# tiantianxuabc/ORB_SLAM2_Refactored

Hardware: AMD Instinct MI355X
Metric: frames/sec ORB extract+match (1280×720, 8 lvl, 1000 feat) + LocalBA iters/sec (higher is better)
Workload: dtype u8; 1 GPU; C2: 1280x720 mono, 8 levels, 2000 features, extract + brute-force Hamming top-2/ratio match of every frame vs its predecessor; width=1280, height=720, nlevels=8, nfeatures=2000, parallelism=8192-frame job sharded over 1 GPU(s), 8192 frames per GPU

## Files before the change

orb_slam2_refactored_amd/csrc/orbx.hip:

```cpp
#include <algorithm>
#include <cfloat>
#include <cmath>
#include <cstring>
#include <mutex>
#include <type_traits>
#include <vector>

#include <hip/hip_ext.h>

#include "common.h"
#include "qt_sort.h"
#include "sincos_f.h"
#include "stereo.h"

namespace orbamd {

constexpr int MAX_LEVELS = 16;
constexpr int MAX_ZONE = 64;
constexpr int MAX_ROOTS = 32;
constexpr int PATCH = 43;
constexpr int HBLUR_W = 37;
constexpr int HBS = 40;
static_assert(HBLUR_W + 3 <= HBS, "the blur's fourth-column tiles store up to column 39");

// ... 2693 lines not shown
        asm volatile("s_waitcnt vmcnt(0) lgkmcnt(0)\n\ts_nop 7\n\ts_nop 7" ::: "memory");
#endif
        const i4v cinit = {128 * 256, 128 * 256, 128 * 256, 128 * 256};
        i4v acc[3][3];
#pragma unroll
        for (int nt = 0; nt < 3; nt++)
#pragma unroll
            for (int mt = 0; mt < 3; mt++)
#if DESC_HBT
                acc[nt][mt] = __builtin_amdgcn_mfma_i32_16x16x64_i8(bfr[nt], afr[mt], cinit, 0, 0, 0);
#else
                acc[nt][mt] = __builtin_amdgcn_mfma_i32_16x16x64_i8(afr[mt], bfr[nt], cinit, 0, 0, 0);
#endif
#if defined(DESC_DIAG_NOPS) && DESC_DIAG_NOPS == 2
        asm volatile("s_waitcnt vmcnt(0) lgkmcnt(0)\n\ts_nop 7\n\ts_nop 7\n\ts_nop 7" ::: "memory");
#endif
#ifdef DESC_KEEPALIVE_DIAG
        asm volatile("" ::"v"(bfr[0]), "v"(bfr[1]), "v"(bfr[2]));
        asm volatile("" ::"v"(afr[0]), "v"(afr[1]), "v"(afr[2]));
#endif
        auto put = [&](int nt, int mt) {
            uint2 pk;
            pk.x = __builtin_amdgcn_perm((uint32_t)acc[nt][mt].y, (uint32_t)acc[nt][mt].x, 0x05040100u);
            pk.y = __builtin_amdgcn_perm((uint32_t)acc[nt][mt].w, (uint32_t)acc[nt][mt].z, 0x05040100u);
#if DESC_HBT
            *reinterpret_cast<uint2*>(&Hb[(16 * mt + n) * HCS + 16 * nt + 4 * lg]) = pk;
#else
            *reinterpret_cast<uint2*>(&Hb[(16 * nt + n) * HBS + 16 * mt + 4 * lg]) = pk;
#endif
        };
#pragma unroll
        for (int nt = 0; nt < 3; nt++) {
            put(nt, 0);
            put(nt, 1);
        }
#if DESC_HBT
        if (n < 8) {
#else
        if (lg < 2) {
#endif
#pragma unroll
            for (int nt = 0; nt < 3; nt++) put(nt, 2);
        }
    }

#if DESC_PAT_EARLY
    float4 pat[4];
#pragma unroll
    for (int r = 0; r < 4; r++) pat[r] = __builtin_bit_cast(float4, tab16(DT_PAT + 1024 * r));
#endif
#if DESC_ANGLE_MFMA && !DESC_ANGLE_FIRST
    {
        i4v au[3], av[3];
#pragma unroll
        for (int nt = 0; nt < 3; nt++) {
            au[nt] = tab16(DT_AN + 1024 * (2 * nt));
            av[nt] = tab16(DT_AN + 1024 * (2 * nt + 1));
        }
        angle_products(au, av);
    }
#endif
    const float angle = fast_atan2_dev((float)m01, (float)m10);
    DESC_STAMP(2);
    __syncthreads();

    const float factorPI = (float)(M_PI / 180.f);
    const float ang = angle * factorPI;
    float a, b;
    DESC_STAMP(3);
#ifdef DESC_SINCOS_COST_DIAG
    a = __cosf(ang);
    b = __sinf(ang);
#else
    if (TRIG) sincosf_glibc(ang, &b, &a);
    else sincos_f2d_k(ang, &b, &a, c_sincos_k);
#endif
    DESC_STAMP(4);
    auto sample = [&](float x, float y) -> int {
        const float dy = rintf(x * b + y * a), dx = rintf(x * a - y * b);
#if DESC_HBT
        const int q = (int)fmaf(dx, (float)HCS, dy + (float)(18 * HCS + 18));
        const uint32_t* cw = reinterpret_cast<const uint32_t*>(Hb) + (q >> 1);
        const uint32_t d0 = cw[0], d1 = cw[1], d2 = cw[2], d3 = cw[3];
        const uint32_t sh = (uint32_t)(q & 1) * 2u;
        const us2 p01 = u2us(__builtin_amdgcn_alignbyte(d1, d0, sh));
        const us2 p23 = u2us(__builtin_amdgcn_alignbyte(d2, d1, sh));
        const us2 p45 = u2us(__builtin_amdgcn_alignbyte(d3, d2, sh));
        const us2 p6x = u2us(__builtin_amdgcn_alignbyte(d3, d3, sh));
        const us2 k01 = {18, 34}, k23 = {48, 56}, k45 = {48, 34}, k6x = {18, 0};
        unsigned acc = __builtin_amdgcn_udot2(p6x, k6x, 1u << 15, false);
        acc = __builtin_amdgcn_udot2(p01, k01, acc, false);
        acc = __builtin_amdgcn_udot2(p23, k23, acc, false);
        acc = __builtin_amdgcn_udot2(p45, k45, acc, false);
        return (int)(acc >> 16);
#else
        const int ob = (int)fmaf(dy, (float)(2 * HBS), fmaf(dx, 2.f, (float)(2 * (18 * HBS + 18))));
        const uint16_t* col = reinterpret_cast<const uint16_t*>(reinterpret_cast<const uint8_t*>(Hb) + ob);
        const us2 p01 = {col[0], col[HBS]}, p23 = {col[2 * HBS], col[3 * HBS]}, p45 = {col[4 * HBS], col[5 * HBS]};
        const us2 k01 = {18, 34}, k23 = {48, 56}, k45 = {48, 34};
        unsigned acc = __builtin_amdgcn_udot2(p01, k01, 18u * col[6 * HBS] + (1u << 15), false);
        acc = __builtin_amdgcn_udot2(p23, k23, acc, false);
        acc = __builtin_amdgcn_udot2(p45, k45, acc, false);
        return (int)(acc >> 16);
#endif
    };
    unsigned long long words[4];
#pragma unroll
    for (int r = 0; r < 4; r++) {
#if DESC_PAT_EARLY
        const float4 q = pat[r];
#else
        const float4 q = __builtin_bit_cast(float4, tab16(DT_PAT + 1024 * r));
#endif
        words[r] = __ballot(sample(q.x, q.y) < sample(q.z, q.w));
    }
    DESC_STAMP(5);
    uint32_t dv = 0, kv = 0;
#pragma unroll
    for (int r = 0; r < 4; r++) {
        dv = writelane_u32((uint32_t)words[r], 2 * r, dv);
        dv = writelane_u32((uint32_t)(words[r] >> 32), 2 * r + 1, dv);
    }
    const float ks = l > 0 ? L.scale : 1.f;
    kv = writelane_u32(__float_as_uint((float)kx * ks), 0, kv);
    kv = writelane_u32(__float_as_uint((float)ky * ks), 1, kv);
    kv = writelane_u32(__float_as_uint(L.size), 2, kv);
    kv = writelane_u32(__float_as_uint(angle), 3, kv);
    kv = writelane_u32(__float_as_uint((float)score), 4, kv);
    kv = writelane_u32((uint32_t)l, 5, kv);
    kv = writelane_u32(0xffffffffu, 6, kv);
    if (lane < 8) reinterpret_cast<uint32_t*>(desc + o * 32)[lane] = dv;
    if (lane < 7) reinterpret_cast<uint32_t*>(kps + o)[lane] = kv;
    DESC_STAMP(6);
}

#ifndef DESC_SLOT_TAB
#define DESC_SLOT_TAB 1
#endif
constexpr int LVP = 32;

__global__ __launch_bounds__(256) void describe_prefix_kernel(const int* __restrict__ sel_cnt, int nl, int F,
                                                              int* __restrict__ lvl_pre, int32_t* __restrict__ counts,
                                                              int* __restrict__ stat) {
    const int f = blockIdx.x * blockDim.x + threadIdx.x;
    if (f >= F) return;
    int acc = 0;
    int* pre = lvl_pre + (long long)f * LVP;
    for (int q = 0; q < nl; q++) {
        pre[q] = acc;
        acc += sel_cnt[f * nl + q];
    }
    pre[nl] = acc;
    counts[f] = acc;
    atomicMax(stat, acc);
}

struct DescGrid {
    int C;
    unsigned m;
    int s1, s2;
};
template <int TRIG>
__device__ __forceinline__ void describe_dense_slot(const Geom& g, int f, int s, const uint8_t* __restrict__ in,
                                                    long long in_fstride, int in_step, const uint8_t* __restrict__ pyr,
                                                    const uint32_t* __restrict__ sel, orbx_keypoint* __restrict__ kps,
                                                    uint8_t* __restrict__ desc, int cap, const int* __restrict__ lvl_pre,
                                                    uint16_t* Hb, int lb) {
    const int lane = threadIdx.x, nl = g.nlevels;
    const int pq = lane <= nl ? lvl_pre[(long long)f * LVP + lane] : 0x7fffffff;
    const int T = __builtin_amdgcn_readlane(pq, nl);
    if (s >= T || s >= cap) return;
    const int l = popc64(__ballot(lane >= 1 && lane <= nl && pq <= s));
    const int pre_l = __builtin_amdgcn_readlane(pq, l);
    const uint32_t k = sel[(long long)f * g.out_frame + g.lv[l].out_base + (s - pre_l)];
    describe_keypoint<TRIG>(g, l, f, k, (long long)f * cap + s, in, in_fstride, in_step, pyr, kps, desc, Hb, lb);
}

template <int TRIG>
__global__ __launch_bounds__(64) void describe_overflow_kernel(Geom g, const uint8_t* __restrict__ in,
                                                               long long in_fstride, int in_step,
                                                               const uint8_t* __restrict__ pyr,
                                                               const uint32_t* __restrict__ sel,
                                                               orbx_keypoint* __restrict__ kps,
                                                               uint8_t* __restrict__ desc, int cap,
                                                               const int* __restrict__ lvl_pre, int F, int C) {
    __shared__ __attribute__((aligned(16))) uint16_t Hb[HB_ELEMS];
    for (int f = blockIdx.x; f < F; f += gridDim.x) {
        const int T = min(lvl_pre[(long long)f * LVP + g.nlevels], cap);
        for (int s = C; s < T; s++) {
            describe_dense_slot<TRIG>(g, f, s, in, in_fstride, in_step, pyr, sel, kps, desc, cap, lvl_pre, Hb,
                                      (int)blockIdx.x);
            __syncthreads();
        }
    }
}

template <int TRIG>
__global__ __launch_bounds__(64) void describe_kernel(Geom g, const uint8_t* __restrict__ in, long long in_fstride,
                                                      int in_step, const uint8_t* __restrict__ pyr,
                                                      const uint32_t* __restrict__ sel,
                                                      const int* __restrict__ sel_cnt, orbx_keypoint* __restrict__ kps,
                                                      uint8_t* __restrict__ desc, int32_t* __restrict__ counts,
                                                      int cap, const uint32_t* __restrict__ slot_tab,
                                                      const int* __restrict__ lvl_pre, DescGrid dg) {
    __shared__ __attribute__((aligned(16))) uint16_t Hb[HB_ELEMS];
    static_assert(47 * RS + 64 <= HB_ELEMS * 2, "R (and the blur's reads of rows 43..47) must fit in Hb");
    const int lane = threadIdx.x;
    const int lb = xcd_swizzle(blockIdx.x + gridDim.x * blockIdx.y, gridDim.x * gridDim.y);
    DESC_STAMP(7);
    if (dg.C > 0) {
        const unsigned t = __umulhi((unsigned)lb, dg.m);
        const int fd = (int)((t + (((unsigned)lb - t) >> dg.s1)) >> dg.s2);
        (void)sel_cnt; (void)counts; (void)slot_tab;
        describe_dense_slot<TRIG>(g, fd, lb - fd * dg.C, in, in_fstride, in_step, pyr, sel, kps, desc, cap, lvl_pre, Hb,
                                  lb);
        return;
    }
    const int f = divmod_of(g, lb);
    const int s = lb - f * g.out_frame;
#if DESC_SLOT_TAB
    (void)sel_cnt;
    (void)counts;
    (void)lane;
    const uint32_t e = slot_tab[s];
    const uint32_t k = sel[(long long)f * g.out_frame + s];
    asm volatile("" ::"s"(e), "s"(k), "s"(cap), "s"(in), "s"(in_fstride), "s"(in_step), "s"(pyr), "s"(g.pyr_frame_bytes));
    const int l = (int)(e & 255u), i = (int)(e >> 8);
    const int2 pr = *reinterpret_cast<const int2*>(lvl_pre + (long long)f * LVP + l);
    {
        const LevelDev& L = g.lv[l];
        asm volatile("" ::"s"(pr.x), "s"(pr.y), "s"(L.w), "s"(L.h), "s"(L.stride), "s"(L.off));
    }
    if (i >= pr.y - pr.x) return;
    const int oidx = pr.x + i;
    if (oidx >= cap) return;
#else
    (void)slot_tab;
    (void)lvl_pre;
    const int nl = g.nlevels;
    const uint32_t k = sel[(long long)f * g.out_frame + s];
    const int* cf = sel_cnt + f * nl;
    int cnt16[MAX_LEVELS];
#pragma unroll
    for (int q = 0; q < MAX_LEVELS; q++) cnt16[q] = cf[q];
    int l = MAX_LEVELS;
    {
        const unsigned s1 = (unsigned)(s + 1) * 0x00010001u;
#pragma unroll
        for (int d = 0; d < MAX_LEVELS / 2; d++) l -= __popc(((g.lv_start[d] | 0x80008000u) - s1) & 0x80008000u);
    }
    int total = 0, lbase = 0, cnt_l = 0;
#pragma unroll
    for (int q = 0; q < MAX_LEVELS; q++) {
        const int cq = q < nl ? cnt16[q] : 0;
        total += cq;
        lbase += q < l ? cq : 0;
        cnt_l = q == l ? cq : cnt_l;
    }
    if (s == 0 && lane == 0) counts[f] = total;
    const int i = s - g.lv[l].out_base;
    if (i >= cnt_l) return;
    const int oidx = lbase + i;
    if (oidx >= cap) return;
#endif
    describe_keypoint<TRIG>(g, l, f, k, (long long)f * cap + oidx, in, in_fstride, in_step, pyr, kps, desc, Hb, lb);
}

__global__ __launch_bounds__(256) void qt_sort_test_kernel(QtItem* items, int n, int* scratch) {
    __shared__ int s_cnt[2];
    qt_sort_block<false>(items, n, scratch, scratch + n, scratch + 2 * n, scratch + 3 * n,
                  reinterpret_cast<QtItem*>(scratch + 4 * n), scratch + 6 * n, n / 3 + 2, s_cnt);
}

}

using namespace orbamd;

struct orbx_extractor {
    orbx_params p;
    int device = 0;
    hipStream_t stream = nullptr;
    std::vector<float> scale, inv_scale, sigma2, inv_sigma2;
    std::vector<int> quota;
    std::mutex mu;

    int g_rows = -1, g_cols = -1;
    Geom geom;
    std::vector<CellDev> cells;
    int NC = 0, PTC = 0;
    size_t qt_lds = 0;
    int qt_ptc0 = 0;
    size_t qt_lds0 = 0;
    int qt_wave = 0, qt_wave_wg = 2, qtw_l0 = 0, qtw_nc = 0, qtw_ptc = 0;
    size_t qtw_lds = 0;
    FastLds fl;
    size_t fast_lds = 0;
    int fast_cpw = 16;
    int fast_spec = 8;
    int fast_pair = 0;
    bool fast_pair_on = false;
    int fast_spec_first = 1;
    int nsub = 1;
    int debug_nc = 0;
    int debug_qt_block = 0;
    uint32_t fault_host = 0;
    int pyr_mfma = 0;
    std::vector<char> pyr_mfma_ok;
    DevBuf d_pyrmt, d_pyrkb;
    int pyr_pair = 2;
    int trig_float = 0;
    int resize_simd = 0;
    std::vector<std::pair<hipStream_t, hipEvent_t>> sub;
    hipEvent_t fork_ev = nullptr;
    bool lvl_overlap = false;
    hipStream_t lvl_side = nullptr;
    hipEvent_t lvl_fork = nullptr, lvl_join = nullptr;
    DevBuf d_cells, d_xtab, d_ytab;
    DevBuf d_strips;
    DevBuf d_slottab;
    DevBuf d_lvlpre;
    std::vector<int> strip_beg;

    int ws_frames = 0;
    DevBuf d_pyr, d_slots, d_cellcnt, d_P, d_T, d_sel, d_selcnt, d_fault;
    DevBuf d_img, d_kps, d_desc, d_counts;
    DevBuf d_stereo_sad;
    int prof = 0;
    std::vector<std::pair<hipEvent_t, hipEvent_t>> prof_ev[4];
    std::vector<hipEvent_t> ev_pool;
    const uint8_t* last_in = nullptr;
    long long last_fstride = 0;
    size_t last_step = 0;
    int last_frames = 0;
    int desc_dense = 0;
    int desc_force_c = 0;
    int desc_c = 0;
    DevBuf d_dstat;
    int32_t* h_dstat = nullptr;
    hipEvent_t dstat_ev = nullptr;
    bool dstat_pending = false;
    bool last_single = false;
    int last_kcap = 0;
    DevBuf d_stereo_out;
    std::vector<uint8_t> h_stage;
};

static int resize_tail_x(int w, int V) {
    if (V <= 0) return w;
    if (V == 1) return 0;
    int x = 0;
    for (; x <= w - V; x += V) {}
    for (; x < w - V / 2; x += V / 2) {}
    return x;
}

static int cv_round_d(double v) { return (int)std::lrint(v); }
static int cv_round_f(float v) { return (int)std::lrintf(v); }

static void compute_tables(orbx_extractor* h) {
    const orbx_params& p = h->p;
    const int L = p.nlevels;
    h->scale.resize(L); h->inv_scale.resize(L); h->sigma2.resize(L); h->inv_sigma2.resize(L);
    h->quota.resize(L);
    float s = 1.f;
    for (int l = 0; l < L; l++) {
        h->scale[l] = s;
        h->inv_scale[l] = 1.f / s;
        h->sigma2[l] = s * s;
        h->inv_sigma2[l] = 1.f / (s * s);
        s *= p.scaleFactor;
    }
    const double factor = 1 / p.scaleFactor;
    double nf = p.nfeatures * (1 - factor) / (1 - std::pow(factor, L));
    int sum = 0;
    for (int l = 0; l < L - 1; l++) {
        h->quota[l] = cv_round_d(nf);
        sum += h->quota[l];
        nf *= factor;
    }
    h->quota[L - 1] = std::max(p.nfeatures - sum, 0);
}

static int setup_geometry(orbx_extractor* h, int rows, int cols) {
    if (h->g_rows == rows && h->g_cols == cols) return ORB_OK;
    const int Lc = h->p.nlevels;
    Geom g;
    std::memset(&g, 0, sizeof(g));
    g.nlevels = Lc;
    for (int l = Lc; l < MAX_LEVELS; l++) g.lv[l].out_base = INT_MAX;
    std::vector<int2> xtab, ytab;
    std::vector<PyrMfmaLane> mt;
    std::vector<int> mkb;
    std::vector<CellDev> cells;
    long long pyr_off = 0, slot = 0, cand = 0;
    int out = 0, NC = 64;
    int prev_w = cols, prev_h = rows;
    for (int l = 0; l < Lc; l++) {
        LevelDev& L = g.lv[l];
        if (l == 0) {
            L.w = cols; L.h = rows; L.stride = cols; L.off = -1; L.tail_x = cols; L.mt_off = -1;
        } else {
            L.h = cv_round_f(h->inv_scale[l] * rows);
            L.w = cv_round_f(h->inv_scale[l] * cols);
            if (L.w <= 0 || L.h <= 0) {
                set_error("pyramid level collapses to zero size");
                return ORB_EINVAL;
            }
            L.stride = (int)align_up(L.w, 16);
            L.off = pyr_off;
            pyr_off += (long long)align_up((size_t)L.stride * L.h, 256);
            const int sw = prev_w, sh = prev_h, dw = L.w, dh = L.h;
            const double scale_x = 1. / ((double)dw / sw), scale_y = 1. / ((double)dh / sh);
            L.xtab_off = (int)xtab.size();
            L.ytab_off = (int)ytab.size();
            L.ssx = (double)sw / L.w;
            L.ssy = (double)sh / L.h;
            L.tail_x = resize_tail_x(L.w, h->resize_simd);
            int xmax = dw;
            std::vector<int> sxs(dw), a0s(dw), a1s(dw);
            for (int dx = 0; dx < dw; dx++) {
                float fx = (float)((dx + 0.5) * scale_x - 0.5);
                int sx = (int)std::floor(fx);
                fx -= sx;
                if (sx < 0) { fx = 0; sx = 0; }
                if (sx + 1 >= sw) {
                    xmax = std::min(xmax, dx);
                    if (sx >= sw - 1) { fx = 0; sx = sw - 1; }
                }
                sxs[dx] = sx;
                a0s[dx] = std::min(std::max(cv_round_f((1.f - fx) * 2048), -32768), 32767);
                a1s[dx] = std::min(std::max(cv_round_f(fx * 2048), -32768), 32767);
            }
            for (int dx = 0; dx < dw; dx++) {
                int sx0 = sxs[dx], sx1 = std::min(sxs[dx] + 1, sw - 1), a0 = a0s[dx], a1 = a1s[dx];
                if (dx >= xmax) { sx1 = sx0; a0 = 2048; a1 = 0; }
                xtab.push_back(make_int2(sx0 | (sx1 << 16), (a0 & 0xffff) | (a1 << 16)));
            }
            L.mt_off = h->pyr_mfma ? pyr_mfma_tables(xtab.data() + L.xtab_off, dw, mt, mkb) : -1;
            for (int dy = 0; dy < dh; dy++) {
                float fy = (float)((dy + 0.5) * scale_y - 0.5);
                int sy = (int)std::floor(fy);
                fy -= sy;
                const int b0 = std::min(std::max(cv_round_f((1.f - fy) * 2048), -32768), 32767);
                const int b1 = std::min(std::max(cv_round_f(fy * 2048), -32768), 32767);
                auto clip = [&](int y) { return y < 0 ? 0 : (y >= sh ? sh - 1 : y); };
                ytab.push_back(make_int2(clip(sy) | (clip(sy + 1) << 16), (b0 & 0xffff) | (b1 << 16)));
            }
        }
        if (l > 0) {
            const double sc = (double)prev_w / L.w, scy = (double)prev_h / L.h;
            if (sc * PYR_TW + 12 > PYR_SW || scy * PYR_TH + 6 > PYR_SH) {
                set_error("scaleFactor too large for the pyramid tile (max ~1.9)");
                return ORB_EINVAL;
            }
        }
        if (L.w >= 4096 || L.h >= 4096) {
            set_error("image dimensions must be < 4096");
            return ORB_EINVAL;
        }
        prev_w = L.w; prev_h = L.h;
        L.rx = 16; L.ry = 16; L.rw = L.w - 32; L.rh = L.h - 32;
        L.scale = h->scale[l];
        L.size = h->scale[l] * 31;
        L.quota = h->quota[l];
        L.cell_base = (int)cells.size();
        L.ncells = 0;
        L.cand_base = cand;
        L.cand_cap = 0;
        L.nroots = 0;
// ... 107 lines not shown
        }
    }
    int rc;
    if ((rc = h->d_cells.reserve(std::max<size_t>(1, cells.size()) * sizeof(CellDev)))) return rc;
    if ((rc = h->d_xtab.reserve(std::max<size_t>(1, xtab.size()) * sizeof(int2)))) return rc;
    if ((rc = h->d_ytab.reserve(std::max<size_t>(1, ytab.size()) * sizeof(int2)))) return rc;
    if (!cells.empty())
        ORB_HIP_TRY(hipMemcpy(h->d_cells.ptr, cells.data(), cells.size() * sizeof(CellDev), hipMemcpyHostToDevice));
    if (!xtab.empty())
        ORB_HIP_TRY(hipMemcpy(h->d_xtab.ptr, xtab.data(), xtab.size() * sizeof(int2), hipMemcpyHostToDevice));
    if (!ytab.empty())
        ORB_HIP_TRY(hipMemcpy(h->d_ytab.ptr, ytab.data(), ytab.size() * sizeof(int2), hipMemcpyHostToDevice));
    {
        std::vector<uint32_t> st((size_t)g.out_frame, 0u);
        for (int l = 0; l < Lc; l++)
            for (int i = 0; i < g.lv[l].out_cap; i++) st[(size_t)g.lv[l].out_base + i] = (uint32_t)l | ((uint32_t)i << 8);
        if ((rc = h->d_slottab.reserve(st.size() * sizeof(uint32_t)))) return rc;
        ORB_HIP_TRY(hipMemcpy(h->d_slottab.ptr, st.data(), st.size() * sizeof(uint32_t), hipMemcpyHostToDevice));
    }
    if (!mt.empty() && (rc = h->d_pyrmt.reserve(mt.size() * sizeof(PyrMfmaLane)))) return rc;
    if (!mkb.empty() && (rc = h->d_pyrkb.reserve(mkb.size() * sizeof(int)))) return rc;
    if (!mt.empty())
        ORB_HIP_TRY(hipMemcpy(h->d_pyrmt.ptr, mt.data(), mt.size() * sizeof(PyrMfmaLane), hipMemcpyHostToDevice));
    if (!mkb.empty())
        ORB_HIP_TRY(hipMemcpy(h->d_pyrkb.ptr, mkb.data(), mkb.size() * sizeof(int), hipMemcpyHostToDevice));
    h->pyr_mfma_ok.assign(Lc, 0);
    for (int l = 1; l + 1 < Lc; l++) h->pyr_mfma_ok[l] = h->pyr_mfma && pyr_mfma_pair_fits(g, l, mkb, ytab);
    h->geom = g;
    h->cells = cells;
    {
        std::vector<int2> strips;
        h->strip_beg.assign(g.nlevels + 1, 0);
        const int cpw = std::max(1, std::min(h->fast_cpw, 255));
        for (int l = 0; l < g.nlevels; l++) {
            h->strip_beg[l] = (int)strips.size();
            const LevelDev& L = g.lv[l];
            if (L.ncells <= 0) continue;
            const int x00 = cells[L.cell_base].x0y0 & 0xffff;
            int ncx = 0;
            while (ncx < L.ncells && (cells[L.cell_base + ncx].x0y0 >> 16) == (cells[L.cell_base].x0y0 >> 16)) ncx++;
            const int ncy = L.ncells / ncx;
            if (ncx * ncy != L.ncells || (cells[L.cell_base + ncx - 1].x0y0 & 0xffff) < x00) {
                set_error("FAST cell grid is not a rectangle");
                return ORB_EINTERNAL;
            }
            for (int rb = 0; rb < ncy; rb += cpw)
                for (int cx = 0; cx < ncx; cx++) {
                    const int c0 = L.cell_base + rb * ncx + cx, n = std::min(cpw, ncy - rb);
                    for (int k = 1; k < n; k++)
                        if ((cells[c0 + k * ncx].zwzh & 0xffff) != (cells[c0].zwzh & 0xffff)) {
                            set_error("FAST strip with unequal zone widths");
                            return ORB_EINTERNAL;
                        }
                    strips.push_back(make_int2(c0, n | (ncx << 8)));
                }
        }
        h->strip_beg[g.nlevels] = (int)strips.size();
        if ((rc = h->d_strips.reserve(std::max<size_t>(1, strips.size()) * sizeof(int2)))) return rc;
        if (!strips.empty())
            ORB_HIP_TRY(hipMemcpy(h->d_strips.ptr, strips.data(), strips.size() * sizeof(int2), hipMemcpyHostToDevice));
    }
    {
        int mzw = 1, mzh = 1;
        for (const CellDev& c : cells) { mzw = std::max(mzw, c.zwzh & 0xffff); mzh = std::max(mzh, c.zwzh >> 16); }
        if (mzw > 64 || mzh > (2 * GR_RING + FQ2_RING) / 8) {
            set_error("FAST cell larger than the kernel supports");
            return ORB_EINTERNAL;
        }
        h->fast_pair_on = false;
        if (h->fast_pair) {
            bool ok = 2 * mzh < 128 && 24 * ((2 * mzh + 1) / (mzw <= 32 ? 2 : 1) + 1) <= 2 * (2 * GR_RING + FQ2_RING);
            for (int l = 0; l < g.nlevels && ok; l++) {
                const LevelDev& L = g.lv[l];
                if (L.ncells <= 0) continue;
                int ncx = 0;
                while (ncx < L.ncells && (cells[L.cell_base + ncx].x0y0 >> 16) == (cells[L.cell_base].x0y0 >> 16)) ncx++;
                for (int c = L.cell_base; c + ncx < L.cell_base + L.ncells && ok; c++) {
                    const CellDev &A = cells[c], &B = cells[c + ncx];
                    ok = (A.x0y0 & 0xffff) == (B.x0y0 & 0xffff) && (B.x0y0 >> 16) == (A.x0y0 >> 16) + (A.zwzh >> 16);
                }
            }
            h->fast_pair_on = ok;
        }
        const int zrows = h->fast_pair_on ? 2 * mzh + 1 : mzh;
        FastLds fl;
        fl.CS = (int)align_up(mzw + 6 + 8, 4);
        if (fl.CS < 4 * ((mzw + 6 + 1 + 3) / 4)) fl.CS = 4 * ((mzw + 6 + 1 + 3) / 4);
        fl.ZS = (int)align_up(mzw + 2, 4);
        fl.crop_bytes = (int)align_up((size_t)fl.CS * std::max(zrows + 6 + FAST_CROP_SLACK, 4 * CROP_NG), 16);
        fl.mz_bytes = (int)align_up((size_t)fl.ZS * (zrows + 2), 16);
        fl.qcap = 2 * GR_RING + FQ2_RING;
        fl.ccap = std::min(FAST_CLIST_CAP, (int)align_up((size_t)mzw * mzh, 8));
        const int nbal = (fl.ccap + 63) / 64;
        h->fast_lds = (size_t)fl.crop_bytes + fl.mz_bytes + 2 * (size_t)(fl.qcap + fl.ccap) +
                      (h->fast_pair_on ? 24 : 16) * (size_t)nbal;
        h->fl = fl;
    }
    h->NC = NC;
    h->PTC = PTC;
    h->qt_lds = lds;
    h->qt_ptc0 = PTC0;
    h->qt_lds0 = lds0;
    h->g_rows = rows;
    h->g_cols = cols;
    h->ws_frames = 0;
    return ORB_OK;
}

static int reserve_workspace(orbx_extractor* h, int frames) {
    if (frames <= h->ws_frames) return ORB_OK;
    const Geom& g = h->geom;
    int rc;
    if ((rc = h->d_pyr.reserve((size_t)frames * g.pyr_frame_bytes))) return rc;
    if ((rc = h->d_slots.reserve((size_t)frames * g.slot_frame * 4))) return rc;
    if ((rc = h->d_cellcnt.reserve((size_t)frames * std::max(1, g.ncells_total) * 4))) return rc;
    if ((rc = h->d_P.reserve((size_t)frames * g.cand_frame * 4))) return rc;
    if ((rc = h->d_T.reserve((size_t)frames * g.cand_frame * 4))) return rc;
    if ((rc = h->d_sel.reserve((size_t)frames * g.out_frame * 4))) return rc;
    if ((rc = h->d_selcnt.reserve((size_t)frames * g.nlevels * 4 + 64))) return rc;
    if ((rc = h->d_lvlpre.reserve((size_t)frames * LVP * 4))) return rc;
    if (!h->d_fault.ptr) {
        if ((rc = h->d_fault.reserve(16))) return rc;
        ORB_HIP_TRY(hipMemset(h->d_fault.ptr, 0, 16));
    }
    h->ws_frames = frames;
    return ORB_OK;
}

static hipEvent_t prof_event(orbx_extractor* h) {
    if (!h->ev_pool.empty()) {
        hipEvent_t e = h->ev_pool.back();
        h->ev_pool.pop_back();
        return e;
    }
    hipEvent_t e = nullptr;
    (void)hipEventCreate(&e);
    return e;
}

constexpr int ORBX_MIN_SUB_FRAMES = 16;

template <typename... KArgs, typename... Args>
static void launch_timed(orbx_extractor* h, int stage, void (*kernel)(KArgs...), dim3 grid, dim3 block,
                         uint32_t shmem, hipStream_t s, Args... args) {
    if (h->prof & (1 << stage)) {
        hipEvent_t a = prof_event(h), b = prof_event(h);
        hipExtLaunchKernelGGL(kernel, grid, block, shmem, s, a, b, 0, static_cast<KArgs>(args)...);
        h->prof_ev[stage].push_back({a, b});
    } else {
        hipLaunchKernelGGL(kernel, grid, block, shmem, s, static_cast<KArgs>(args)...);
    }
}

static void launch_chunk(orbx_extractor* h, int f0, const uint8_t* d_imgs, int F, long long fstride, int step,
                         orbx_keypoint* d_kps, uint8_t* d_desc, int32_t* d_counts, int cap, hipStream_t st,
                         hipStream_t side = nullptr) {
    const Geom& g = h->geom;
    uint8_t* pyr = h->d_pyr.as<uint8_t>() + (long long)f0 * g.pyr_frame_bytes;
    d_imgs += (long long)f0 * fstride;
    d_kps += (long long)f0 * cap;
    d_desc += (long long)f0 * cap * 32;
    d_counts += f0;
    uint32_t* slots = h->d_slots.as<uint32_t>() + (long long)f0 * g.slot_frame;
    int* cellcnt = h->d_cellcnt.as<int>() + (long long)f0 * g.ncells_total;
    uint32_t* Pb = h->d_P.as<uint32_t>() + (long long)f0 * g.cand_frame;
    uint32_t* Tb = h->d_T.as<uint32_t>() + (long long)f0 * g.cand_frame;
    uint32_t* sel = h->d_sel.as<uint32_t>() + (long long)f0 * g.out_frame;
    int* selcnt = h->d_selcnt.as<int>() + (long long)f0 * g.nlevels;
    uint32_t* fault = h->d_fault.as<uint32_t>();
    auto fast = [&](int l0, int l1, hipStream_t s) {
        const int sb = h->strip_beg[l0], ns = h->strip_beg[l1] - sb;
        if (ns <= 0) return;
        const FastLds& fl = h->fl;
        auto kern = h->fast_pair_on ? (fl.CS == 48 && fl.ZS == 36   ? fast_cells_kernel<48, 36, true>
                                       : fl.CS == 52 && fl.ZS == 40 ? fast_cells_kernel<52, 40, true>
                                                                    : fast_cells_kernel<0, 0, true>)
                                    : (fl.CS == 48 && fl.ZS == 36   ? fast_cells_kernel<48, 36, false>
                                       : fl.CS == 52 && fl.ZS == 40 ? fast_cells_kernel<52, 40, false>
                                                                    : fast_cells_kernel<0, 0, false>);
        launch_timed(h, 1, kern, dim3((unsigned)(ns * F)), dim3(64), (uint32_t)h->fast_lds, s,
                           g, h->d_cells.as<CellDev>(), h->d_strips.as<int2>(), d_imgs, fstride, step, pyr, h->p.iniThFAST,
                           h->p.minThFAST, slots, cellcnt, fault, h->fl, sb, ns,
                           h->fast_spec > 0 && h->fast_spec_first ? h->fast_spec | (1 << 29) : h->fast_spec);
    };
    const unsigned qt_block = h->debug_qt_block ? (unsigned)h->debug_qt_block : (unsigned)QT_THREADS;
    auto quadtree = [&](int l0, int nl, hipStream_t s) {
        if (nl <= 0) return;
        const int lw = std::max(l0, h->qtw_l0), nw_lv = l0 + nl - lw;
        if (nw_lv > 0) {
            launch_timed(h, 2, quadtree_kernel<true>, dim3((unsigned)F, (unsigned)((nw_lv + 3) / 4)), dim3(qt_block),
                         (uint32_t)h->qtw_lds, s, g, cellcnt, slots, h->d_cells.as<CellDev>(), Pb, Tb, sel, selcnt, h->qtw_nc,
                         h->qtw_ptc, fault, lw, nw_lv);
            nl -= nw_lv;
            if (nl <= 0) return;
        }
        if (h->qt_ptc0 > 0 && l0 == 0) {
            launch_timed(h, 2, quadtree_kernel<false>, dim3((unsigned)F, 1u), dim3(qt_block), (uint32_t)h->qt_lds0, s, g,
                         cellcnt, slots, h->d_cells.as<CellDev>(), Pb, Tb, sel, selcnt, h->NC, h->qt_ptc0, fault, 0, 1);
            l0 = 1;
            if (--nl <= 0) return;
        }
        launch_timed(h, 2, quadtree_kernel<false>, dim3((unsigned)F, (unsigned)nl), dim3(qt_block), (uint32_t)h->qt_lds, s,
                     g, cellcnt, slots, h->d_cells.as<CellDev>(), Pb, Tb, sel, selcnt, h->NC, h->PTC, fault, l0, nl);
    };
    auto pyramid = [&](int l) -> int {
        const int first = h->pyr_pair == 2 ? 1 : 2;
        const bool a16 = l > 1 || (((uintptr_t)d_imgs | (uintptr_t)fstride | (uintptr_t)step) & 15) == 0;
        if (h->pyr_pair && l >= first && (l - first) % 2 == 0 && l + 1 < g.nlevels && a16 && h->pyr_mfma &&
            h->pyr_mfma_ok[l]) {
            const int ntx = (g.lv[l + 1].w + PYR_TW - 1) / PYR_TW, nty = (g.lv[l + 1].h + PYR_TH - 1) / PYR_TH;
            launch_timed(h, 0, pyramid_pair_mfma_kernel, dim3((unsigned)ntx, (unsigned)nty, (unsigned)F), dim3(256), 0u,
                         st, g, l, d_imgs, fstride, step, pyr, h->d_ytab.as<int2>(), h->d_pyrmt.as<PyrMfmaLane>(),
                         h->d_pyrkb.as<int>());
            return 1;
        }
        if (h->pyr_pair && l >= first && (l - first) % 2 == 0 && l + 1 < g.nlevels && a16 && pyr_pair_fits(g, l)) {
            const int ntx = (g.lv[l + 1].w + PYR_TW - 1) / PYR_TW, nty = (g.lv[l + 1].h + PYR_TH - 1) / PYR_TH;
            launch_timed(h, 0, pyramid_pair_kernel, dim3((unsigned)ntx, (unsigned)nty, (unsigned)F), dim3(256), 0u, st,
                         g, l, d_imgs, fstride, step, pyr, h->d_xtab.as<int2>(), h->d_ytab.as<int2>());
            return 1;
        }
        const int ntx = (g.lv[l].w + PYR_TW - 1) / PYR_TW, nty = (g.lv[l].h + PYR_TH - 1) / PYR_TH;
        launch_timed(h, 0, pyramid_level_kernel, dim3((unsigned)ntx, (unsigned)nty, (unsigned)F), dim3(256), 0u, st, g, l,
                     d_imgs, fstride, step, pyr, h->d_xtab.as<int2>(), h->d_ytab.as<int2>());
        return 0;
    };
    const int nc0 = g.lv[0].ncells;
    if (side && nc0 > 0 && g.nlevels > 1) {
        (void)hipStreamWaitEvent(side, h->lvl_fork, 0);
        fast(0, 1, side);
        quadtree(0, 1, side);
        (void)hipEventRecord(h->lvl_join, side);
        {
            for (int l = 1; l < g.nlevels; l++) l += pyramid(l);
        }
        fast(1, g.nlevels, st);
        quadtree(1, g.nlevels - 1, st);
        (void)hipStreamWaitEvent(st, h->lvl_join, 0);
    } else {
        {
            for (int l = 1; l < g.nlevels; l++) l += pyramid(l);
        }
        fast(0, g.nlevels, st);
        quadtree(0, g.nlevels, st);
    }
    int* lvlpre = h->d_lvlpre.as<int>() + (long long)f0 * LVP;
    if (DESC_SLOT_TAB)
        hipLaunchKernelGGL(describe_prefix_kernel, dim3((unsigned)((F + 255) / 256)), dim3(256), 0, st, (const int*)selcnt,
                           g.nlevels, F, lvlpre, d_counts, h->d_dstat.as<int>());
    const int rows_max = std::min(g.out_frame, cap);
    const int C = (DESC_SLOT_TAB && h->desc_dense) ? std::max(1, std::min(h->desc_c > 0 ? h->desc_c : rows_max, rows_max)) : 0;
    DescGrid dg{};
    if (C > 0) {
        dg.C = C;
        const unsigned d = (unsigned)C;
        int lg = 0;
        while ((1ull << lg) < d) lg++;
        dg.m = (unsigned)((((1ull << lg) - d) << 32) / d + 1);
        dg.s1 = lg > 0 ? 1 : 0;
        dg.s2 = lg > 0 ? lg - 1 : 0;
    }
    launch_timed(h, 3, h->trig_float ? describe_kernel<1> : describe_kernel<0>,
                 dim3((unsigned)(C > 0 ? C : g.out_frame), (unsigned)F), dim3(64), 0u, st, g, d_imgs, fstride, step, pyr,
                 sel, selcnt, d_kps, d_desc, d_counts, cap, h->d_slottab.as<uint32_t>(), lvlpre, dg);
    if (C > 0 && C < rows_max)
        launch_timed(h, 3, h->trig_float ? describe_overflow_kernel<1> : describe_overflow_kernel<0>,
                     dim3((unsigned)std::min(F, 2048)), dim3(64), 0u, st, g, d_imgs, fstride, step, pyr, sel, d_kps, d_desc,
                     cap, (const int*)lvlpre, F, C);
}

static int launch_fast_hint(orbx_extractor* h, hipStream_t st) {
    if (!(h->fast_spec > 0 && h->fast_spec_first)) return ORB_OK;
    const int ns = h->strip_beg[h->geom.nlevels];
    if (ns <= 0) return ORB_OK;
    hipLaunchKernelGGL(fast_hint_kernel, dim3((unsigned)((ns + 255) / 256)), dim3(256), 0, st, h->d_strips.as<int2>(),
                       h->d_cellcnt.as<int>(), ns);
    ORB_HIP_TRY(hipGetLastError());
    return ORB_OK;
}

static int describe_grid_begin(orbx_extractor* h, hipStream_t st) {
    if (!h->dstat_ev) {
        ORB_HIP_TRY(hipEventCreateWithFlags(&h->dstat_ev, hipEventDisableTiming));
        ORB_HIP_TRY(hipHostMalloc((void**)&h->h_dstat, 64, hipHostMallocDefault));
        int rc;
        if ((rc = h->d_dstat.reserve(64))) return rc;
    }
    if (h->dstat_pending && hipEventQuery(h->dstat_ev) == hipSuccess) {
        const int mx = *h->h_dstat;
        h->desc_c = (int)align_up((size_t)std::max(mx + 32, 64), 64);
        h->dstat_pending = false;
    }
    if (h->desc_force_c > 0) h->desc_c = h->desc_force_c;
    ORB_HIP_TRY(hipMemsetAsync(h->d_dstat.ptr, 0, 4, st));
    return ORB_OK;
}
static int describe_grid_end(orbx_extractor* h, hipStream_t st) {
    if (h->dstat_pending) return ORB_OK;
    ORB_HIP_TRY(hipMemcpyAsync(h->h_dstat, h->d_dstat.ptr, 4, hipMemcpyDeviceToHost, st));
    ORB_HIP_TRY(hipEventRecord(h->dstat_ev, st));
    h->dstat_pending = true;
    return ORB_OK;
}

static int launch_batch(orbx_extractor* h, const uint8_t* d_imgs, int F, long long fstride, int step,
                        orbx_keypoint* d_kps, uint8_t* d_desc, int32_t* d_counts, int cap, hipStream_t st) {
    {
        const int rc = describe_grid_begin(h, st);
        if (rc) return rc;
    }
    int nsub = std::min(h->nsub, F / ORBX_MIN_SUB_FRAMES);
    if (nsub <= 1) {
        hipStream_t side = nullptr;
        if (h->lvl_overlap) {
            if (!h->lvl_side) {
                ORB_HIP_TRY(hipStreamCreateWithFlags(&h->lvl_side, hipStreamNonBlocking));
                ORB_HIP_TRY(hipEventCreateWithFlags(&h->lvl_fork, hipEventDisableTiming));
                ORB_HIP_TRY(hipEventCreateWithFlags(&h->lvl_join, hipEventDisableTiming));
            }
            ORB_HIP_TRY(hipEventRecord(h->lvl_fork, st));
            side = h->lvl_side;
        }
        launch_chunk(h, 0, d_imgs, F, fstride, step, d_kps, d_desc, d_counts, cap, st, side);
        ORB_HIP_TRY(hipGetLastError());
        const int rc = describe_grid_end(h, st);
        return rc ? rc : launch_fast_hint(h, st);
    }
    while ((int)h->sub.size() < nsub) {
        hipStream_t s2;
        ORB_HIP_TRY(hipStreamCreateWithFlags(&s2, hipStreamNonBlocking));
        hipEvent_t e;
        ORB_HIP_TRY(hipEventCreateWithFlags(&e, hipEventDisableTiming));
        h->sub.push_back({s2, e});
    }
    if (!h->fork_ev) ORB_HIP_TRY(hipEventCreateWithFlags(&h->fork_ev, hipEventDisableTiming));
    ORB_HIP_TRY(hipEventRecord(h->fork_ev, st));
    int f0 = 0;
    for (int i = 0; i < nsub; i++) {
        const int Fi = F / nsub + (i < F % nsub ? 1 : 0);
        ORB_HIP_TRY(hipStreamWaitEvent(h->sub[i].first, h->fork_ev, 0));
        launch_chunk(h, f0, d_imgs, Fi, fstride, step, d_kps, d_desc, d_counts, cap, h->sub[i].first);
        ORB_HIP_TRY(hipEventRecord(h->sub[i].second, h->sub[i].first));
        ORB_HIP_TRY(hipStreamWaitEvent(st, h->sub[i].second, 0));
        f0 += Fi;
    }
    ORB_HIP_TRY(hipGetLastError());
    const int rc = describe_grid_end(h, st);
    return rc ? rc : launch_fast_hint(h, st);
}

static int check_fault(orbx_extractor* h) {
    uint32_t f = 0;
    ORB_HIP_TRY(hipMemcpy(&f, h->d_fault.ptr, 4, hipMemcpyDeviceToHost));
    if (f) {
        ORB_HIP_TRY(hipMemset(h->d_fault.ptr, 0, 4));
        set_error("device capacity check failed (fault mask " + std::to_string(f) + ")");
        return ORB_EINTERNAL;
    }
    return ORB_OK;
}

namespace orbamd {
__global__ __launch_bounds__(256) void pack_rows_kernel(const uint4* __restrict__ desc, int cap,
                                                        const int* __restrict__ counts, const int* __restrict__ incl,
                                                        uint4* __restrict__ out, int out_rows) {
    const int f = blockIdx.x;
    const int c = counts[f];
    const int n = min(max(c, 0), cap);
    const long long start = (long long)incl[f] - c;
    const long long r0 = max(start, 0ll), r1 = min(start + n, (long long)out_rows);
    const uint4* src = desc + (long long)f * cap * 2;
    for (long long i = 2 * r0 + threadIdx.x; i < 2 * r1; i += blockDim.x) out[i] = src[i - 2 * start];
}

}

extern "C" {

int orbx_create(const orbx_params* params, int device, orbx_extractor** out) {
    ORB_CHECK_ARG(params && out, "null argument");
    ORB_CHECK_ARG(params->nlevels >= 1 && params->nlevels <= MAX_LEVELS, "nlevels must be in [1,16]");
    ORB_CHECK_ARG(params->nfeatures >= 0 && params->scaleFactor > 1.0f, "bad nfeatures / scaleFactor");
    int ndev = 0;
    ORB_HIP_TRY(hipGetDeviceCount(&ndev));
    ORB_CHECK_ARG(device >= 0 && device < ndev, "no such HIP device");
    ORB_HIP_TRY(hipSetDevice(device));
    orbx_extractor* h = new orbx_extractor();
    h->p = *params;
    h->device = device;
    if (const char* e = getenv("ORBX_FAST_CPW")) h->fast_cpw = std::max(1, std::min(64, atoi(e)));
    if (const char* e = getenv("ORBX_FAST_SPEC")) h->fast_spec = std::max(-1, atoi(e));
    if (const char* e = getenv("ORBX_FAST_PAIR")) h->fast_pair = atoi(e) != 0;
    if (const char* e = getenv("ORBX_QT_WAVE")) h->qt_wave = atoi(e) != 0;
    if (const char* e = getenv("ORBX_QT_WAVE_WG")) h->qt_wave_wg = std::max(1, std::min(4, atoi(e)));
    if (const char* e = getenv("ORBX_FAST_SPEC_FIRST")) h->fast_spec_first = atoi(e) != 0;

    if (const char* e = getenv("ORBX_NSUB")) h->nsub = std::max(1, std::min(8, atoi(e)));
    if (const char* e = getenv("ORBX_PYR_PAIR")) h->pyr_pair = std::max(0, std::min(2, atoi(e)));
    if (const char* e = getenv("ORBX_PYR_MFMA")) h->pyr_mfma = atoi(e) != 0;
    if (const char* e = getenv("ORBX_LEVEL_OVERLAP")) h->lvl_overlap = atoi(e) != 0;
    if (const char* e = getenv("ORBX_DEBUG_NC")) h->debug_nc = atoi(e);
    if (const char* e = getenv("ORBX_DESC_DENSE")) h->desc_dense = atoi(e) != 0;
    if (const char* e = getenv("ORBX_DESC_C")) h->desc_force_c = std::max(0, atoi(e));
    if (const char* e = getenv("ORBX_DEBUG_QT_BLOCK")) {
        const int b = atoi(e);
        if (b >= 64 && b <= QT_THREADS && b % 64 == 0) h->debug_qt_block = b;
    }
    if (const char* e = getenv("ORBX_TRIG")) h->trig_float = (e[0] == 'f' || e[0] == '1') ? 1 : 0;
    if (const char* e = getenv("ORBX_RESIZE_TAIL")) {
        const int v = atoi(e);
        if (v == 0 || v == 1 || v == 8 || v == 16 || v == 32 || v == 64) h->resize_simd = v;
    }
    compute_tables(h);
    hipError_t e = hipStreamCreateWithFlags(&h->stream, hipStreamNonBlocking);
    if (e != hipSuccess) {
        delete h;
        set_error(std::string("hipStreamCreate: ") + hipGetErrorString(e));
        return ORB_EHIP;
    }
    *out = h;
    return ORB_OK;
}

int orbx_destroy(orbx_extractor* h) {
    if (!h) return ORB_OK;
    (void)hipSetDevice(h->device);
    DevBuf* bufs[] = {&h->d_cells, &h->d_strips, &h->d_xtab, &h->d_ytab, &h->d_pyr, &h->d_slots, &h->d_cellcnt, &h->d_P,
                      &h->d_T, &h->d_sel, &h->d_selcnt, &h->d_fault, &h->d_img, &h->d_kps, &h->d_desc,
                      &h->d_counts, &h->d_stereo_sad, &h->d_pyrmt, &h->d_pyrkb, &h->d_slottab, &h->d_lvlpre,
                      &h->d_stereo_out, &h->d_dstat};
    for (DevBuf* b : bufs) b->release();
    for (auto& v : h->prof_ev)
        for (auto& pr : v) { (void)hipEventDestroy(pr.first); (void)hipEventDestroy(pr.second); }
    for (hipEvent_t e : h->ev_pool) (void)hipEventDestroy(e);
    if (h->stream) (void)hipStreamDestroy(h->stream);
    for (auto& se : h->sub) { (void)hipStreamDestroy(se.first); (void)hipEventDestroy(se.second); }
    if (h->fork_ev) (void)hipEventDestroy(h->fork_ev);
    if (h->lvl_side) (void)hipStreamDestroy(h->lvl_side);
    if (h->lvl_fork) (void)hipEventDestroy(h->lvl_fork);
    if (h->lvl_join) (void)hipEventDestroy(h->lvl_join);
    if (h->dstat_ev) (void)hipEventDestroy(h->dstat_ev);
    if (h->h_dstat) (void)hipHostFree(h->h_dstat);
    delete h;
    return ORB_OK;
}

int orbx_set_opencv_compat(orbx_extractor* h, int trig_mode, int resize_simd) {
    ORB_CHECK_ARG(h, "null extractor");
    ORB_CHECK_ARG(trig_mode >= -1 && trig_mode <= 1, "trig_mode must be -1 (keep), 0 (double) or 1 (float)");
    ORB_CHECK_ARG(resize_simd == -1 || resize_simd == 0 || resize_simd == 1 || resize_simd == 8 || resize_simd == 16 ||
                      resize_simd == 32 || resize_simd == 64,
                  "resize_simd must be -1 (keep), 0, 1, 8, 16, 32 or 64");
    std::lock_guard<std::mutex> lk(h->mu);
    if (trig_mode >= 0) h->trig_float = trig_mode;
    if (resize_simd >= 0 && resize_simd != h->resize_simd) {
        h->resize_simd = resize_simd;
        h->g_rows = h->g_cols = -1;
    }
    return ORB_OK;
}

int orbx_get_opencv_compat(const orbx_extractor* h, int* trig_mode, int* resize_simd) {
    ORB_CHECK_ARG(h, "null extractor");
    if (trig_mode) *trig_mode = h->trig_float;
    if (resize_simd) *resize_simd = h->resize_simd;
    return ORB_OK;
}

int orbx_scale_tables(const orbx_extractor* h, float* scale, float* inv_scale, float* sigma2, float* inv_sigma2,
                      int32_t* features_per_level) {
    ORB_CHECK_ARG(h, "null extractor");
    for (int l = 0; l < h->p.nlevels; l++) {
        if (scale) scale[l] = h->scale[l];
        if (inv_scale) inv_scale[l] = h->inv_scale[l];
        if (sigma2) sigma2[l] = h->sigma2[l];
        if (inv_sigma2) inv_sigma2[l] = h->inv_sigma2[l];
        if (features_per_level) features_per_level[l] = h->quota[l];
    }
    return ORB_OK;
}

int orbx_max_keypoints(const orbx_extractor* hc, int rows, int cols, int32_t* cap) {
    ORB_CHECK_ARG(hc && cap && rows > 0 && cols > 0, "bad argument");
    orbx_extractor* h = const_cast<orbx_extractor*>(hc);
    std::lock_guard<std::mutex> lk(h->mu);
    ORB_HIP_TRY(hipSetDevice(h->device));
    int rc = setup_geometry(h, rows, cols);
    if (rc) return rc;
    int c = 0;
    for (int l = 0; l < h->geom.nlevels; l++) c += h->geom.lv[l].out_cap;
    *cap = c;
    return ORB_OK;
}

int orbx_extract_batch_device(orbx_extractor* h, const uint8_t* d_imgs, int n_frames, int rows, int cols,
                              size_t frame_stride, size_t step, orbx_keypoint* d_kps, uint8_t* d_desc,
                              int32_t* d_counts, int cap, void* stream) {
    ORB_CHECK_ARG(h && d_imgs && d_kps && d_desc && d_counts, "null argument");
    ORB_CHECK_ARG(n_frames > 0 && n_frames <= 65535 && rows > 0 && cols > 0, "bad batch shape");
    ORB_CHECK_ARG(step >= (size_t)cols && step < (1u << 31), "bad row step");
    std::lock_guard<std::mutex> lk(h->mu);
    ORB_HIP_TRY(hipSetDevice(h->device));
    int rc = setup_geometry(h, rows, cols);
    if (rc) return rc;
    int need = 0;
    for (int l = 0; l < h->geom.nlevels; l++) need += h->geom.lv[l].out_cap;
    if (cap < need) {
        set_error("cap < orbx_max_keypoints()");
        return ORB_ECAP;
    }
    if ((rc = reserve_workspace(h, n_frames))) return rc;
    hipStream_t st = (hipStream_t)stream;
    h->last_in = d_imgs;
    h->last_single = false;
    h->last_fstride = (long long)frame_stride;
    h->last_step = step;
    h->last_frames = n_frames;
    return launch_batch(h, d_imgs, n_frames, (long long)frame_stride, (int)step, d_kps, d_desc, d_counts, cap, st);
}

int orbx_extract(orbx_extractor* h, const uint8_t* img, int rows, int cols, size_t step, orbx_keypoint* kps,
                 uint8_t* desc, int cap, int* n) {
    ORB_CHECK_ARG(h && img && n, "null argument");
    ORB_CHECK_ARG(rows > 0 && cols > 0 && step >= (size_t)cols, "image must be a non-empty CV_8U matrix");
    std::lock_guard<std::mutex> lk(h->mu);
    ORB_HIP_TRY(hipSetDevice(h->device));
    int rc = setup_geometry(h, rows, cols);
    if (rc) return rc;
    int kcap = 0;
    for (int l = 0; l < h->geom.nlevels; l++) kcap += h->geom.lv[l].out_cap;
    if ((rc = reserve_workspace(h, 1))) return rc;
    if ((rc = h->d_img.reserve((size_t)rows * cols))) return rc;
    if ((rc = h->d_kps.reserve((size_t)kcap * sizeof(orbx_keypoint)))) return rc;
    if ((rc = h->d_desc.reserve((size_t)kcap * 32))) return rc;
    if ((rc = h->d_counts.reserve(16))) return rc;
    hipStream_t st = h->stream;
    if (step == (size_t)cols)
        ORB_HIP_TRY(hipMemcpyAsync(h->d_img.ptr, img, (size_t)rows * cols, hipMemcpyHostToDevice, st));
    else
        ORB_HIP_TRY(hipMemcpy2DAsync(h->d_img.ptr, cols, img, step, cols, rows, hipMemcpyHostToDevice, st));
    h->last_in = h->d_img.as<uint8_t>();
    h->last_fstride = (long long)rows * cols;
    h->last_step = cols;
    h->last_frames = 1;
    h->last_single = true;
    h->last_kcap = kcap;
    rc = launch_batch(h, h->d_img.as<uint8_t>(), 1, (long long)rows * cols, cols, h->d_kps.as<orbx_keypoint>(),
                      h->d_desc.as<uint8_t>(), h->d_counts.as<int32_t>(), kcap, st);
    if (rc) return rc;
    int32_t total = 0;
    ORB_HIP_TRY(hipMemcpyAsync(&total, h->d_counts.ptr, 4, hipMemcpyDeviceToHost, st));
    ORB_HIP_TRY(hipStreamSynchronize(st));
    if ((rc = check_fault(h))) return rc;
    *n = total;
    if (total == 0) return ORB_OK;
    if (total > cap) {
        set_error("output capacity too small");
        return ORB_ECAP;
    }
    ORB_CHECK_ARG(kps && desc, "null output");
    ORB_HIP_TRY(hipMemcpyAsync(kps, h->d_kps.ptr, (size_t)total * sizeof(orbx_keypoint), hipMemcpyDeviceToHost, st));
    ORB_HIP_TRY(hipMemcpyAsync(desc, h->d_desc.ptr, (size_t)total * 32, hipMemcpyDeviceToHost, st));
    ORB_HIP_TRY(hipStreamSynchronize(st));
    return ORB_OK;
}

int orbx_batch_status(orbx_extractor* h, void* stream, uint32_t* fault_mask) {
    ORB_CHECK_ARG(h && fault_mask, "null argument");
    std::lock_guard<std::mutex> lk(h->mu);
    ORB_HIP_TRY(hipSetDevice(h->device));
    *fault_mask = 0;
    if (!h->d_fault.ptr) return ORB_OK;
    hipStream_t st = (hipStream_t)stream;
    ORB_HIP_TRY(hipMemcpyAsync(&h->fault_host, h->d_fault.ptr, 4, hipMemcpyDeviceToHost, st));
    ORB_HIP_TRY(hipMemsetAsync(h->d_fault.ptr, 0, 4, st));
    ORB_HIP_TRY(hipStreamSynchronize(st));
    *fault_mask = h->fault_host;
    if (h->fault_host) {
        set_error("device capacity check failed in a batch (fault mask " + std::to_string(h->fault_host) + ")");
        return ORB_EINTERNAL;
    }
    return ORB_OK;
}

int orbx_fault_word_device(orbx_extractor* h, uint32_t** d_fault) {
    ORB_CHECK_ARG(h && d_fault, "null argument");
    std::lock_guard<std::mutex> lk(h->mu);
    ORB_HIP_TRY(hipSetDevice(h->device));
    int rc;
    if (!h->d_fault.ptr) {
        if ((rc = h->d_fault.reserve(16))) return rc;
        ORB_HIP_TRY(hipMemset(h->d_fault.ptr, 0, 16));
    }
// ... 275 lines not shown
```

Before: 176,800 frames/s.

## Add optional two-stream chunked pipeline splitting detect and describe stages

Adds an opt-in mode that splits the frame batch into chunks and runs pyramid/FAST on a front stream while quadtree and descriptor stages of earlier chunks run on a back stream, linked by per-chunk events. The goal is to overlap the stages across chunks so the GPU stays busy. It also skips the max-count atomic and the host readback of descriptor stats when dense describe is off. The pipeline adds event and stream overhead and reorders the stage launches inside launch_chunk.

Result: no change. 176,900 frames/s, median of 2 (+0.1%).

```diff
diff --git a/orb_slam2_refactored_amd/csrc/orbx.hip b/orb_slam2_refactored_amd/csrc/orbx.hip
--- a/orb_slam2_refactored_amd/csrc/orbx.hip
+++ b/orb_slam2_refactored_amd/csrc/orbx.hip
@@ -2869,7 +2869,7 @@
     }
     pre[nl] = acc;
     counts[f] = acc;
-    atomicMax(stat, acc);
+    if (stat) atomicMax(stat, acc);
 }
 
 struct DescGrid {
@@ -3032,6 +3032,13 @@
     bool lvl_overlap = false;
     hipStream_t lvl_side = nullptr;
     hipEvent_t lvl_fork = nullptr, lvl_join = nullptr;
+    int pipe = 0;
+    int pipe_chunk = 1024;
+    int pipe_prio = 0;
+    int pipe_qt_front = 0;
+    hipStream_t pipe_front = nullptr, pipe_back = nullptr;
+    hipEvent_t pipe_fork = nullptr, pipe_done = nullptr;
+    std::vector<hipEvent_t> pipe_ev;
     DevBuf d_cells, d_xtab, d_ytab;
     DevBuf d_strips;
     DevBuf d_slottab;
@@ -3445,9 +3452,11 @@
     }
 }
 
+enum : int { CHUNK_FAST = 1, CHUNK_QT = 2, CHUNK_DESC = 4, CHUNK_ALL = 7 };
+
 static void launch_chunk(orbx_extractor* h, int f0, const uint8_t* d_imgs, int F, long long fstride, int step,
                          orbx_keypoint* d_kps, uint8_t* d_desc, int32_t* d_counts, int cap, hipStream_t st,
-                         hipStream_t side = nullptr) {
+                         hipStream_t side = nullptr, int parts = CHUNK_ALL) {
     const Geom& g = h->geom;
     uint8_t* pyr = h->d_pyr.as<uint8_t>() + (long long)f0 * g.pyr_frame_bytes;
     d_imgs += (long long)f0 * fstride;
@@ -3520,27 +3529,30 @@
     };
     const int nc0 = g.lv[0].ncells;
     if (side && nc0 > 0 && g.nlevels > 1) {
-        (void)hipStreamWaitEvent(side, h->lvl_fork, 0);
-        fast(0, 1, side);
-        quadtree(0, 1, side);
-        (void)hipEventRecord(h->lvl_join, side);
-        {
+        if (parts & CHUNK_FAST) {
+            (void)hipStreamWaitEvent(side, h->lvl_fork, 0);
+            fast(0, 1, side);
             for (int l = 1; l < g.nlevels; l++) l += pyramid(l);
-        }
-        fast(1, g.nlevels, st);
-        quadtree(1, g.nlevels - 1, st);
-        (void)hipStreamWaitEvent(st, h->lvl_join, 0);
+            fast(1, g.nlevels, st);
+        }
+        if (parts & CHUNK_QT) {
+            quadtree(0, 1, side);
+            (void)hipEventRecord(h->lvl_join, side);
+            quadtree(1, g.nlevels - 1, st);
+            (void)hipStreamWaitEvent(st, h->lvl_join, 0);
+        }
     } else {
-        {
+        if (parts & CHUNK_FAST) {
             for (int l = 1; l < g.nlevels; l++) l += pyramid(l);
-        }
-        fast(0, g.nlevels, st);
-        quadtree(0, g.nlevels, st);
-    }
+            fast(0, g.nlevels, st);
+        }
+        if (parts & CHUNK_QT) quadtree(0, g.nlevels, st);
+    }
+    if (!(parts & CHUNK_DESC)) return;
     int* lvlpre = h->d_lvlpre.as<int>() + (long long)f0 * LVP;
     if (DESC_SLOT_TAB)
         hipLaunchKernelGGL(describe_prefix_kernel, dim3((unsigned)((F + 255) / 256)), dim3(256), 0, st, (const int*)selcnt,
-                           g.nlevels, F, lvlpre, d_counts, h->d_dstat.as<int>());
+                           g.nlevels, F, lvlpre, d_counts, h->desc_dense ? h->d_dstat.as<int>() : nullptr);
     const int rows_max = std::min(g.out_frame, cap);
     const int C = (DESC_SLOT_TAB && h->desc_dense) ? std::max(1, std::min(h->desc_c > 0 ? h->desc_c : rows_max, rows_max)) : 0;
     DescGrid dg{};
@@ -3573,6 +3585,7 @@
 }
 
 static int describe_grid_begin(orbx_extractor* h, hipStream_t st) {
+    if (!h->desc_dense) return ORB_OK;
     if (!h->dstat_ev) {
         ORB_HIP_TRY(hipEventCreateWithFlags(&h->dstat_ev, hipEventDisableTiming));
         ORB_HIP_TRY(hipHostMalloc((void**)&h->h_dstat, 64, hipHostMallocDefault));
@@ -3589,6 +3602,7 @@
     return ORB_OK;
 }
 static int describe_grid_end(orbx_extractor* h, hipStream_t st) {
+    if (!h->desc_dense) return ORB_OK;
     if (h->dstat_pending) return ORB_OK;
     ORB_HIP_TRY(hipMemcpyAsync(h->h_dstat, h->d_dstat.ptr, 4, hipMemcpyDeviceToHost, st));
     ORB_HIP_TRY(hipEventRecord(h->dstat_ev, st));
@@ -3596,11 +3610,58 @@
     return ORB_OK;
 }
 
+constexpr int ORBX_MAX_PIPE_CHUNKS = 64;
+
+static int pipe_chunks(const orbx_extractor* h, int F) {
+    if (!h->pipe || (h->prof && h->pipe < 2)) return 1;
+    return std::min(F / h->pipe_chunk, ORBX_MAX_PIPE_CHUNKS);
+}
+
+static int launch_batch_pipelined(orbx_extractor* h, int n, const uint8_t* d_imgs, int F, long long fstride, int step,
+                                  orbx_keypoint* d_kps, uint8_t* d_desc, int32_t* d_counts, int cap, hipStream_t st) {
+    if (!h->pipe_front) {
+        int least = 0, greatest = 0;
+        ORB_HIP_TRY(hipDeviceGetStreamPriorityRange(&least, &greatest));
+        ORB_HIP_TRY(hipStreamCreateWithPriority(&h->pipe_front, hipStreamNonBlocking, h->pipe_prio < 0 ? greatest : 0));
+        ORB_HIP_TRY(hipStreamCreateWithPriority(&h->pipe_back, hipStreamNonBlocking, h->pipe_prio > 0 ? greatest : 0));
+        ORB_HIP_TRY(hipEventCreateWithFlags(&h->pipe_fork, hipEventDisableTiming));
+        ORB_HIP_TRY(hipEventCreateWithFlags(&h->pipe_done, hipEventDisableTiming));
+    }
+    while ((int)h->pipe_ev.size() < n) {
+        hipEvent_t e;
+        ORB_HIP_TRY(hipEventCreateWithFlags(&e, hipEventDisableTiming));
+        h->pipe_ev.push_back(e);
+    }
+    const int front = CHUNK_FAST | (h->pipe_qt_front ? CHUNK_QT : 0), back = CHUNK_ALL & ~front;
+    ORB_HIP_TRY(hipEventRecord(h->pipe_fork, st));
+    ORB_HIP_TRY(hipStreamWaitEvent(h->pipe_front, h->pipe_fork, 0));
+    ORB_HIP_TRY(hipStreamWaitEvent(h->pipe_back, h->pipe_fork, 0));
+    int f0 = 0;
+    for (int k = 0; k < n; k++) {
+        const int Fk = F / n + (k < F % n ? 1 : 0);
+        launch_chunk(h, f0, d_imgs, Fk, fstride, step, d_kps, d_desc, d_counts, cap, h->pipe_front, nullptr, front);
+        ORB_HIP_TRY(hipEventRecord(h->pipe_ev[k], h->pipe_front));
+        ORB_HIP_TRY(hipStreamWaitEvent(h->pipe_back, h->pipe_ev[k], 0));
+        launch_chunk(h, f0, d_imgs, Fk, fstride, step, d_kps, d_desc, d_counts, cap, h->pipe_back, nullptr, back);
+        f0 += Fk;
+    }
+    ORB_HIP_TRY(hipEventRecord(h->pipe_done, h->pipe_back));
+    ORB_HIP_TRY(hipStreamWaitEvent(st, h->pipe_ev[n - 1], 0));
+    ORB_HIP_TRY(hipStreamWaitEvent(st, h->pipe_done, 0));
+    ORB_HIP_TRY(hipGetLastError());
+    return ORB_OK;
+}
+
 static int launch_batch(orbx_extractor* h, const uint8_t* d_imgs, int F, long long fstride, int step,
                         orbx_keypoint* d_kps, uint8_t* d_desc, int32_t* d_counts, int cap, hipStream_t st) {
     {
         const int rc = describe_grid_begin(h, st);
         if (rc) return rc;
+    }
+    if (const int n = pipe_chunks(h, F); n >= 2) {
+        int rc = launch_batch_pipelined(h, n, d_imgs, F, fstride, step, d_kps, d_desc, d_counts, cap, st);
+        if (!rc) rc = describe_grid_end(h, st);
+        return rc ? rc : launch_fast_hint(h, st);
     }
     int nsub = std::min(h->nsub, F / ORBX_MIN_SUB_FRAMES);
     if (nsub <= 1) {
@@ -3692,6 +3753,10 @@
     if (const char* e = getenv("ORBX_PYR_PAIR")) h->pyr_pair = std::max(0, std::min(2, atoi(e)));
     if (const char* e = getenv("ORBX_PYR_MFMA")) h->pyr_mfma = atoi(e) != 0;
     if (const char* e = getenv("ORBX_LEVEL_OVERLAP")) h->lvl_overlap = atoi(e) != 0;
+    if (const char* e = getenv("ORBX_PIPE")) h->pipe = std::max(0, std::min(2, atoi(e)));
+    if (const char* e = getenv("ORBX_PIPE_CHUNK")) h->pipe_chunk = std::max(1, std::min(65535, atoi(e)));
+    if (const char* e = getenv("ORBX_PIPE_PRIO")) h->pipe_prio = std::max(-1, std::min(1, atoi(e)));
+    if (const char* e = getenv("ORBX_PIPE_QT_FRONT")) h->pipe_qt_front = atoi(e) != 0;
     if (const char* e = getenv("ORBX_DEBUG_NC")) h->debug_nc = atoi(e);
     if (const char* e = getenv("ORBX_DESC_DENSE")) h->desc_dense = atoi(e) != 0;
     if (const char* e = getenv("ORBX_DESC_C")) h->desc_force_c = std::max(0, atoi(e));
@@ -3732,6 +3797,11 @@
     if (h->lvl_side) (void)hipStreamDestroy(h->lvl_side);
     if (h->lvl_fork) (void)hipEventDestroy(h->lvl_fork);
     if (h->lvl_join) (void)hipEventDestroy(h->lvl_join);
+    if (h->pipe_front) (void)hipStreamDestroy(h->pipe_front);
+    if (h->pipe_back) (void)hipStreamDestroy(h->pipe_back);
+    if (h->pipe_fork) (void)hipEventDestroy(h->pipe_fork);
+    if (h->pipe_done) (void)hipEventDestroy(h->pipe_done);
+    for (hipEvent_t e : h->pipe_ev) (void)hipEventDestroy(e);
     if (h->dstat_ev) (void)hipEventDestroy(h->dstat_ev);
     if (h->h_dstat) (void)hipHostFree(h->h_dstat);
     delete h;
```
